# syzhang092218-source/dgppo

Hardware: AMD Instinct MI355X
Metric: env-steps/sec whole node, LidarSpread n=8 4096 envs, 1/2/4/8 GPUs (higher is better)
Workload: dtype f32

## Files before the change

### dgppo_amd/csrc/nn_dense.hip

```cpp
#include "common.h"
#include "nn_gru.h"

using f32x4 = __attribute__((ext_vector_type(4))) float;
#ifdef DGPPO_STAMPS
__device__ unsigned long long g_dstamps[32];
#define DSTAMP(i) do { if (blockIdx.x == 0 && threadIdx.x == 0) g_dstamps[i] = __builtin_amdgcn_s_memtime(); } while (0)
extern "C" int32_t dgppo_debug_stamps_dense(unsigned long long* out) {
  return (int32_t)hipMemcpyFromSymbol(out, HIP_SYMBOL(g_dstamps), sizeof(unsigned long long) * 32);
}
#else
#define DSTAMP(i)
#endif

#define DENSE_ROWS 64

struct DenseArgs {
  const float* X; int ldx;
  const float* W; int ldw;
  const float* bias;
  float* Y; int ldy;
  int M, K, N;
  int act;
  int accumulate;
  int trans_w;
// ... 201 lines not shown
    }
  } else {
    for (; tile < n_tiles; tile += gridDim.x) {
      stage_scalar(tile, 0);
      load_yold(tile);
      __syncthreads();
      compute(0);
      epilogue(tile);
      DGPPO_LDS_BARRIER();
    }
  }
#undef DGPPO_LDS_BARRIER
  DSTAMP(2);
}

template <int NTW, int RTW, int CG, int KQ, bool ACC>
static void launch_dense_acc(const DenseArgs& a, hipStream_t s) {
  constexpr int RB = 16 * RTW * (4 / CG);
  constexpr size_t smem = 2 * (size_t)RB * (KQ * 16 + 2) * sizeof(float);
  static_assert(smem <= 160 * 1024, "dense tile exceeds the 160 KB LDS of a gfx950 CU");
  static thread_local int cap = 0;
  if (cap == 0) {
    int per_cu = 0, dev = 0, cus = 256;
    if (smem > 64 * 1024)
      (void)hipFuncSetAttribute(reinterpret_cast<const void*>(&dense_fwd_kernel<NTW, RTW, CG, KQ, ACC>),
                                hipFuncAttributeMaxDynamicSharedMemorySize, (int)smem);
    if (hipOccupancyMaxActiveBlocksPerMultiprocessor(&per_cu, reinterpret_cast<const void*>(
            &dense_fwd_kernel<NTW, RTW, CG, KQ, ACC>), 256, smem) != hipSuccess || per_cu < 1) per_cu = 1;
    if (hipGetDevice(&dev) != hipSuccess ||
        hipDeviceGetAttribute(&cus, hipDeviceAttributeMultiprocessorCount, dev) != hipSuccess || cus < 1) cus = 256;
    cap = per_cu * cus;
  }
  const int n_tiles = cdiv(a.M, RB);
  const int grid = n_tiles < cap ? n_tiles : cap;
  hipLaunchKernelGGL((dense_fwd_kernel<NTW, RTW, CG, KQ, ACC>), dim3(grid), dim3(256), smem, s, a);
}

template <int NTW, int RTW, int CG, int KQ>
static void launch_dense_kq(const DenseArgs& a, hipStream_t s) {
  if (a.accumulate) launch_dense_acc<NTW, RTW, CG, KQ, true>(a, s);
  else launch_dense_acc<NTW, RTW, CG, KQ, false>(a, s);
}

template <int NTW, int RTW, int CG>
static void launch_dense(const DenseArgs& a, hipStream_t s) {
  const int kq = cdiv(a.K, 16);
  if (kq <= 1) launch_dense_kq<NTW, RTW, CG, 1>(a, s);
  else if (kq == 2) launch_dense_kq<NTW, RTW, CG, 2>(a, s);
  else if (kq == 3) launch_dense_kq<NTW, RTW, CG, 3>(a, s);
  else if (kq == 4) launch_dense_kq<NTW, RTW, CG, 4>(a, s);
  else if (kq <= 6) launch_dense_kq<NTW, RTW, CG, 6>(a, s);
  else if (kq <= 8) launch_dense_kq<NTW, RTW, CG, 8>(a, s);
  else if (kq == 9) launch_dense_kq<NTW, RTW, CG, 9>(a, s);
  else if (kq <= 12) launch_dense_kq<NTW, RTW, CG, 12>(a, s);
  else launch_dense_kq<NTW, RTW, CG, 16>(a, s);
}

#define DSK_MAXK 16
template <bool VECY>
__global__ void __launch_bounds__(256) dense_smallk_kernel(DenseArgs a) {
  __shared__ float sW[DSK_MAXK * 192 + 192];
  const int K = a.K, N = a.N, nq = (N + 3) >> 2, Nl = nq * 4;
  for (int idx = threadIdx.x; idx < K * Nl; idx += 256) {
    const int k = idx / Nl, c = idx - k * Nl;
    float w = 0.0f;
    if (c < N) w = a.trans_w ? a.W[(size_t)c * a.ldw + k] : a.W[(size_t)k * a.ldw + c];
    sW[idx] = w;
  }
  for (int c = threadIdx.x; c < Nl; c += 256) sW[K * Nl + c] = (a.bias && c < N) ? a.bias[c] : 0.0f;
  __syncthreads();
  const long items = (long)a.M * nq;
  const uint32_t rcp = (uint32_t)((0x100000000ull + nq - 1) / nq);
  for (long it = (long)blockIdx.x * 256 + threadIdx.x; it < items; it += (long)gridDim.x * 256) {
    const int row = (int)__umulhi((uint32_t)it, rcp);
    const int c0 = ((int)it - row * nq) * 4;
    const float* x = a.X + (size_t)row * a.ldx;
    float4 acc = *reinterpret_cast<const float4*>(sW + K * Nl + c0);
    for (int k = 0; k < K; ++k) {
      const float xv = x[k];
      const float4 w = *reinterpret_cast<const float4*>(sW + k * Nl + c0);
      acc.x = fmaf(xv, w.x, acc.x); acc.y = fmaf(xv, w.y, acc.y); acc.z = fmaf(xv, w.z, acc.z); acc.w = fmaf(xv, w.w, acc.w);
    }
    float* y = a.Y + (size_t)row * a.ldy + c0;
    float r[4] = {acc.x, acc.y, acc.z, acc.w};
    if (VECY) {
      if (a.accumulate) { const float4 o = *reinterpret_cast<const float4*>(y); r[0] += o.x; r[1] += o.y; r[2] += o.z; r[3] += o.w; }
      if (a.act == 1) { r[0] = relu_nan(r[0]); r[1] = relu_nan(r[1]); r[2] = relu_nan(r[2]); r[3] = relu_nan(r[3]); }
      if (a.mask) {
        const float4 mk = *reinterpret_cast<const float4*>(a.mask + (size_t)row * a.ldm + c0);
        r[0] = mk.x > 0.f ? r[0] : 0.f; r[1] = mk.y > 0.f ? r[1] : 0.f; r[2] = mk.z > 0.f ? r[2] : 0.f; r[3] = mk.w > 0.f ? r[3] : 0.f;
      }
      *reinterpret_cast<float4*>(y) = make_float4(r[0], r[1], r[2], r[3]);
    } else {
      for (int u = 0; u < 4; ++u) {
        if (c0 + u >= N) break;
        float v = r[u];
        if (a.accumulate) v += y[u];
        if (a.act == 1) v = relu_nan(v);
        if (a.mask) v = a.mask[(size_t)row * a.ldm + c0 + u] > 0.f ? v : 0.f;
        y[u] = v;
      }
    }
  }
}

static bool dense_smallk_ok(const DenseArgs& a) {
  const long nq = (a.N + 3) / 4;
  return a.K <= DSK_MAXK && a.N <= 192 && (long)a.M * nq * nq < (1l << 32);
}
static void launch_dense_smallk(const DenseArgs& a, hipStream_t s) {
  const long items = (long)a.M * ((a.N + 3) / 4);
  long blocks = (items + 256 * 4 - 1) / (256 * 4);
  blocks = blocks < 1 ? 1 : (blocks > 4096 ? 4096 : blocks);
  const bool vec = (a.N & 3) == 0 && (a.ldy & 3) == 0 && (reinterpret_cast<uintptr_t>(a.Y) & 15) == 0 &&
                   (!a.mask || ((a.ldm & 3) == 0 && (reinterpret_cast<uintptr_t>(a.mask) & 15) == 0));
  if (vec) hipLaunchKernelGGL(dense_smallk_kernel<true>, dim3((int)blocks), dim3(256), 0, s, a);
  else hipLaunchKernelGGL(dense_smallk_kernel<false>, dim3((int)blocks), dim3(256), 0, s, a);
}

int32_t dense_fwd_launch(const DenseArgs& a, hipStream_t s) {
  DGPPO_REQUIRE(a.M >= 0 && a.K >= 1 && a.N >= 1, "dense: bad shape M=%d K=%d N=%d", a.M, a.K, a.N);
  DGPPO_REQUIRE(a.N <= 192 && a.K <= 256, "dense: N <= 192 and K <= 256 supported (N=%d K=%d)", a.N, a.K);
  DGPPO_REQUIRE(a.X && a.W && a.Y, "dense: NULL operand");
  DGPPO_REQUIRE(a.ldx >= a.K && a.ldy >= a.N, "dense: leading dimensions too small");
  if (a.M == 0) return 0;
  const int nt = cdiv(a.N, 16);
  if (dense_smallk_ok(a)) launch_dense_smallk(a, s);
  else if (nt >= 9) launch_dense<3, 2, 4>(a, s);
  else if (nt >= 5) launch_dense<2, 2, 4>(a, s);
  else if (nt == 4) launch_dense<1, 2, 4>(a, s);
  else if (nt == 3) launch_dense<2, 1, 2>(a, s);
  else if (nt == 2) launch_dense<1, 1, 2>(a, s);
  else launch_dense<1, 1, 1>(a, s);
  DGPPO_LAUNCH_CHECK();
  return 0;
}

struct DenseBwdWArgs {
  const float* X; int ldx;
  const float* dY; int ldy;
  float* dW; int ldw;
  float* db;
  int M, K, N;
  int rows_per_block;
  float* part;
  int part_stride;
  size_t ws_bytes;
  const float* W; int ldwp;
  float* dX; int lddx;
  int acc_mask;
};

#define BW_ROWS 32
template <int NT, int KT, int NG, bool DX = false>
__global__ void __launch_bounds__(256 * NG) dense_bwd_w_kernel(DenseBwdWArgs a) {
  extern __shared__ float sm_wg[];
  constexpr int KTW = (KT + 3) / 4;
  constexpr int Kl = (KT & 1) ? KT * 16 : KT * 16 + 16;
  constexpr int Nl = (NT & 1) ? NT * 16 : NT * 16 + 16;
  constexpr int BUF = BW_ROWS * (Kl + Nl);
  constexpr int XQ = KT * 4, YQ = NT * 4;
  constexpr int PFX = (BW_ROWS * XQ + 255) / 256, PFY = (BW_ROWS * YQ + 255) / 256;
  const int K = a.K, N = a.N;
  const int grp = NG > 1 ? (int)(threadIdx.x >> 8) : 0;
  const int tid = threadIdx.x & 255, lane = tid & 63, wave = tid >> 6;
  const int li = lane & 15, lq = lane >> 4;
  float* sm = sm_wg + grp * 2 * BUF;
  const int wg_begin = blockIdx.x * NG * a.rows_per_block;
  const int m_begin = wg_begin + grp * a.rows_per_block;
  const int m_end = min(a.M, m_begin + a.rows_per_block);
  const int n_tiles = (min(a.M - wg_begin, a.rows_per_block) + BW_ROWS - 1) / BW_ROWS;
  const bool vec = ((K & 3) == 0) && ((a.ldx & 3) == 0) && ((reinterpret_cast<uintptr_t>(a.X) & 15) == 0) &&
                   ((N & 3) == 0) && ((a.ldy & 3) == 0) && ((reinterpret_cast<uintptr_t>(a.dY) & 15) == 0);
  const int K4 = K >> 2, N4 = N >> 2;
  f32x4 acc[KTW][NT];
#pragma unroll
  for (int i = 0; i < KTW; ++i)
#pragma unroll
    for (int t = 0; t < NT; ++t) acc[i][t] = f32x4{0.f, 0.f, 0.f, 0.f};
  float4 pfx[PFX], pfy[PFY], csum[PFY];
#pragma unroll
  for (int u = 0; u < PFY; ++u) csum[u] = make_float4(0.f, 0.f, 0.f, 0.f);
  float4 wreg[DX ? KTW : 1][DX ? NT : 1], ya[DX ? 2 : 1][DX ? NT : 1];
  if constexpr (DX) {
#pragma unroll
    for (int i = 0; i < KTW; ++i) {
      int kt = (3 - wave) + 4 * i;
      kt = kt < KT ? kt : KT - 1;
#pragma unroll
      for (int s = 0; s < NT; ++s)
        wreg[i][s] = *reinterpret_cast<const float4*>(a.W + (size_t)(kt * 16 + li) * a.ldwp + 16 * s + 4 * lq);
    }
  }
  auto fetch_a = [&](int m0) {
    if constexpr (DX) {
#pragma unroll
      for (int mt = 0; mt < 2; ++mt) {
        int row = m0 + mt * 16 + li;
        row = row < a.M ? row : a.M - 1;
#pragma unroll
        for (int s = 0; s < NT; ++s) ya[mt][s] = *reinterpret_cast<const float4*>(a.dY + (size_t)row * a.ldy + 16 * s + 4 * lq);
      }
    }
  };
  auto dx_tile = [&](int m0, int b) {
    if constexpr (DX) {
      const float* xs = sm + b * BUF;
#pragma unroll
      for (int i = 0; i < KTW; ++i) {
        const int kt = (3 - wave) + 4 * i;
        if (kt >= KT) continue;
        const int col = kt * 16 + li;
        float old[2][4];
        if (a.acc_mask) {
#pragma unroll
          for (int mt = 0; mt < 2; ++mt)
#pragma unroll
            for (int r = 0; r < 4; ++r) {
              int row = m0 + mt * 16 + lq * 4 + r;
              row = row < m_end ? row : m_end - 1;
              old[mt][r] = a.dX[(size_t)row * a.lddx + col];
            }
        }
#pragma unroll
        for (int mt = 0; mt < 2; ++mt) {
          f32x4 dx = f32x4{0.f, 0.f, 0.f, 0.f};
#pragma unroll
          for (int s = 0; s < NT; ++s) {
            dx = __builtin_amdgcn_mfma_f32_16x16x4f32(ya[mt][s].x, wreg[i][s].x, dx, 0, 0, 0);
            dx = __builtin_amdgcn_mfma_f32_16x16x4f32(ya[mt][s].y, wreg[i][s].y, dx, 0, 0, 0);
            dx = __builtin_amdgcn_mfma_f32_16x16x4f32(ya[mt][s].z, wreg[i][s].z, dx, 0, 0, 0);
            dx = __builtin_amdgcn_mfma_f32_16x16x4f32(ya[mt][s].w, wreg[i][s].w, dx, 0, 0, 0);
          }
#pragma unroll
          for (int r = 0; r < 4; ++r) {
            const int rl = mt * 16 + lq * 4 + r;
            float v = dx[r];
            if (a.acc_mask) {
              v += old[mt][r];
              v = (xs[rl * Kl + col] > 0.0f) ? v : 0.0f;
            }
            if (m0 + rl < m_end) a.dX[(size_t)(m0 + rl) * a.lddx + col] = v;
          }
        }
      }
    }
  };

  auto fetch = [&](int m0) {
#pragma unroll
    for (int u = 0; u < PFX; ++u) {
      int idx = u * 256 + tid;
      idx = idx < BW_ROWS * XQ ? idx : BW_ROWS * XQ - 1;
      const int r = idx / XQ, q = idx - r * XQ;
      int row = m0 + r;
      row = row < a.M ? row : a.M - 1;
      pfx[u] = *reinterpret_cast<const float4*>(a.X + (size_t)row * a.ldx + 4 * (q < K4 ? q : K4 - 1));
    }
#pragma unroll
    for (int u = 0; u < PFY; ++u) {
      int idx = u * 256 + tid;
      idx = idx < BW_ROWS * YQ ? idx : BW_ROWS * YQ - 1;
      const int r = idx / YQ, q = idx - r * YQ;
      int row = m0 + r;
      row = row < a.M ? row : a.M - 1;
      pfy[u] = *reinterpret_cast<const float4*>(a.dY + (size_t)row * a.ldy + 4 * (q < N4 ? q : N4 - 1));
    }
  };
  auto commit = [&](int m0, int b) {
    float* xs = sm + b * BUF;
    float* ys = xs + BW_ROWS * Kl;
#pragma unroll
    for (int u = 0; u < PFX; ++u) {
      const int idx = u * 256 + tid;
      const int r = idx / XQ, q = idx - r * XQ;
      const bool ok = (m0 + r < m_end) && (q < K4);
      const float4 v = ok ? pfx[u] : make_float4(0.f, 0.f, 0.f, 0.f);
      if (idx < BW_ROWS * XQ) *reinterpret_cast<float4*>(xs + r * Kl + 4 * q) = v;
    }
#pragma unroll
    for (int u = 0; u < PFY; ++u) {
      const int idx = u * 256 + tid;
      const int r = idx / YQ, q = idx - r * YQ;
      const bool ok = (m0 + r < m_end) && (q < N4) && (idx < BW_ROWS * YQ);
      const float4 v = ok ? pfy[u] : make_float4(0.f, 0.f, 0.f, 0.f);
      if (idx < BW_ROWS * YQ) *reinterpret_cast<float4*>(ys + r * Nl + 4 * q) = v;
      csum[u].x += v.x; csum[u].y += v.y; csum[u].z += v.z; csum[u].w += v.w;
    }
  };
  auto stage_scalar = [&](int m0) {
    float* xs = sm;
    float* ys = xs + BW_ROWS * Kl;
    for (int idx = tid; idx < BW_ROWS * KT * 16; idx += 256) {
      const int r = idx / (KT * 16), k = idx - r * (KT * 16);
      xs[r * Kl + k] = (m0 + r < m_end && k < K) ? a.X[(size_t)(m0 + r) * a.ldx + k] : 0.0f;
    }
    for (int idx = tid; idx < BW_ROWS * NT * 16; idx += 256) {
      const int r = idx / (NT * 16), c = idx - r * (NT * 16);
      ys[r * Nl + c] = (m0 + r < m_end && c < N) ? a.dY[(size_t)(m0 + r) * a.ldy + c] : 0.0f;
    }
  };
  auto compute = [&](int b) {
    const float* xs = sm + b * BUF + lq * Kl + li;
    const float* ys = sm + b * BUF + BW_ROWS * Kl + lq * Nl + li;
#pragma unroll
    for (int s4 = 0; s4 < BW_ROWS / 4; ++s4) {
      float bv[NT], av[KTW];
#pragma unroll
      for (int t = 0; t < NT; ++t) bv[t] = ys[s4 * 4 * Nl + t * 16];
#pragma unroll
      for (int i = 0; i < KTW; ++i) {
        int kt = wave + 4 * i;
        kt = kt < KT ? kt : KT - 1;
        av[i] = xs[s4 * 4 * Kl + kt * 16];
      }
#pragma unroll
      for (int i = 0; i < KTW; ++i)
#pragma unroll
        for (int t = 0; t < NT; ++t) acc[i][t] = __builtin_amdgcn_mfma_f32_16x16x4f32(av[i], bv[t], acc[i][t], 0, 0, 0);
    }
  };
#define DGPPO_LDS_BARRIER() asm volatile("s_waitcnt lgkmcnt(0)\n\ts_barrier" ::: "memory")
  float colsum = 0.0f;
  if (DX || vec) {
    fetch(m_begin);
    commit(m_begin, 0);
    __syncthreads();
    int cur = 0;
    for (int it = 0, m0 = m_begin; it < n_tiles; ++it, m0 += BW_ROWS) {
      fetch_a(m0);
      fetch(m0 + BW_ROWS);
      __builtin_amdgcn_sched_barrier(0);
      compute(cur);
      commit(m0 + BW_ROWS, cur ^ 1);
      dx_tile(m0, cur);
      DGPPO_LDS_BARRIER();
      cur ^= 1;
    }
  } else {
    for (int it = 0, m0 = m_begin; it < n_tiles; ++it, m0 += BW_ROWS) {
      stage_scalar(m0);
      __syncthreads();
      if (a.db != nullptr && tid < N) {
        const float* ys = sm + BW_ROWS * Kl;
        float cs = 0.0f;
#pragma unroll 8
        for (int r = 0; r < BW_ROWS; ++r) cs += ys[r * Nl + tid];
        colsum += cs;
      }
      compute(0);
      __syncthreads();
    }
  }
#undef DGPPO_LDS_BARRIER
  if (NG > 1) {
    constexpr int ACCF = KTW * NT * 4 * 256;
    static_assert(NG == 1 || ACCF + PFY * 4 * 256 <= 2 * BUF, "dense_bwd_w: the group exchange does not fit the tile buffers");
    __syncthreads();
    if (grp > 0) {
#pragma unroll
      for (int i = 0; i < KTW; ++i)
#pragma unroll
        for (int t = 0; t < NT; ++t)
#pragma unroll
          for (int r = 0; r < 4; ++r) sm[((i * NT + t) * 4 + r) * 256 + tid] = acc[i][t][r];
      if (!vec) csum[0].x = colsum;
#pragma unroll
      for (int u = 0; u < PFY; ++u) {
        sm[ACCF + (u * 4 + 0) * 256 + tid] = csum[u].x; sm[ACCF + (u * 4 + 1) * 256 + tid] = csum[u].y;
        sm[ACCF + (u * 4 + 2) * 256 + tid] = csum[u].z; sm[ACCF + (u * 4 + 3) * 256 + tid] = csum[u].w;
      }
    }
    __syncthreads();
    if (grp == 0) {
      for (int g = 1; g < NG; ++g) {
        const float* o = sm_wg + g * 2 * BUF;
#pragma unroll
        for (int i = 0; i < KTW; ++i)
#pragma unroll
          for (int t = 0; t < NT; ++t)
#pragma unroll
            for (int r = 0; r < 4; ++r) acc[i][t][r] += o[((i * NT + t) * 4 + r) * 256 + tid];
        if (!vec) colsum += o[ACCF + tid];
        else {
#pragma unroll
          for (int u = 0; u < PFY; ++u) {
            csum[u].x += o[ACCF + (u * 4 + 0) * 256 + tid]; csum[u].y += o[ACCF + (u * 4 + 1) * 256 + tid];
            csum[u].z += o[ACCF + (u * 4 + 2) * 256 + tid]; csum[u].w += o[ACCF + (u * 4 + 3) * 256 + tid];
          }
        }
      }
    }
  }
  float* slab = a.part ? a.part + (size_t)blockIdx.x * a.part_stride : nullptr;
#pragma unroll
  for (int i = 0; i < KTW; ++i) {
    const int kt = wave + 4 * i;
    if (kt >= KT || grp != 0) continue;
#pragma unroll
    for (int t = 0; t < NT; ++t) {
      const int col = t * 16 + li;
      if (col >= N) continue;
#pragma unroll
      for (int r = 0; r < 4; ++r) {
        const int krow = kt * 16 + lq * 4 + r;
        if (krow >= K) continue;
        if (slab) slab[krow * N + col] = acc[i][t][r];
        else atomicAdd(a.dW + (size_t)krow * a.ldw + col, acc[i][t][r]);
      }
    }
  }
  if (a.db != nullptr) {
    float cs = colsum;
    if (vec) {
      __syncthreads();
      float* red = sm;
#pragma unroll
      for (int u = 0; u < PFY; ++u) {
        const int idx = u * 256 + tid;
        const int r = idx / YQ, q = idx - r * YQ;
        if (idx < BW_ROWS * YQ) *reinterpret_cast<float4*>(red + r * (YQ * 4) + 4 * q) = csum[u];
      }
      __syncthreads();
      cs = 0.0f;
      if (tid < N) {
#pragma unroll 8
        for (int r = 0; r < BW_ROWS; ++r) cs += red[r * (YQ * 4) + tid];
      }
    }
    if (tid < N && grp == 0) {
      if (slab) slab[K * N + tid] = cs;
      else atomicAdd(a.db + tid, cs);
    }
  }
}

#define REDUCE_SLABS_PER_SPLIT 16

__global__ void __launch_bounds__(256) dense_bwd_w_reduce_kernel(const float* __restrict__ part, int part_stride, int G,
                                                                 float* __restrict__ dW, int ldw, float* __restrict__ db,
                                                                 int K, int N) {
  const int e = blockIdx.x * 256 + threadIdx.x;
  const int E = K * N + (db ? N : 0);
  if (e >= E) return;
  const int per = (G + gridDim.y - 1) / gridDim.y;
  const int g0 = blockIdx.y * per, g1 = min(G, g0 + per);
  float s0 = 0.f, s1 = 0.f, s2 = 0.f, s3 = 0.f;
  int g = g0;
  for (; g + 3 < g1; g += 4) {
    s0 += part[(size_t)g * part_stride + e];
    s1 += part[(size_t)(g + 1) * part_stride + e];
    s2 += part[(size_t)(g + 2) * part_stride + e];
    s3 += part[(size_t)(g + 3) * part_stride + e];
  }
  for (; g < g1; ++g) s0 += part[(size_t)g * part_stride + e];
  const float sum = (s0 + s1) + (s2 + s3);
  if (g0 >= g1) return;
  if (e < K * N) {
    const int k = e / N, n = e - k * N;
    atomicAdd(dW + (size_t)k * ldw + n, sum);
  } else {
    atomicAdd(db + (e - K * N), sum);
  }
}

static thread_local dgppo_reduce_desc* g_defer = nullptr;

struct ReduceBatch {
  int n;
  dgppo_reduce_desc d[DGPPO_REDUCE_BATCH];
};

__global__ void __launch_bounds__(256) dense_bwd_w_reduce_batch_kernel(ReduceBatch b) {
  const dgppo_reduce_desc& d = b.d[blockIdx.z];
  const int K = d.K, N = d.N, G = d.slabs;
  const int e = blockIdx.x * 256 + threadIdx.x;
  const int E = K * N + (d.db ? N : 0);
  if (e >= E) return;
  const int splits = min((int)gridDim.y, max(1, (G + REDUCE_SLABS_PER_SPLIT - 1) / REDUCE_SLABS_PER_SPLIT));
  if ((int)blockIdx.y >= splits) return;
  const int per = (G + splits - 1) / splits;
  const int g0 = blockIdx.y * per, g1 = min(G, g0 + per);
  if (g0 >= g1) return;
  const float* part = d.part;
  const size_t st = (size_t)d.part_stride;
  float s0 = 0.f, s1 = 0.f, s2 = 0.f, s3 = 0.f;
  int g = g0;
  for (; g + 3 < g1; g += 4) {
    s0 += part[(size_t)g * st + e]; s1 += part[(size_t)(g + 1) * st + e];
    s2 += part[(size_t)(g + 2) * st + e]; s3 += part[(size_t)(g + 3) * st + e];
  }
  for (; g < g1; ++g) s0 += part[(size_t)g * st + e];
  const float sum = (s0 + s1) + (s2 + s3);
  if (e < K * N) {
    const int k = e / N, n = e - k * N;
    atomicAdd(d.dW + (size_t)k * d.ldw + n, sum);
  } else {
    atomicAdd(d.db + (e - K * N), sum);
  }
}

static void reduce_or_defer(hipStream_t s, const float* part, int stride, int grid, float* dW, int ldw, float* db, int K, int N) {
  if (g_defer != nullptr) {
    dgppo_reduce_desc& d = *g_defer;
    d.part = part; d.part_stride = stride; d.slabs = grid; d.dW = dW; d.ldw = ldw; d.db = db; d.K = K; d.N = N; d.pending = 1;
    return;
  }
  const int E = K * N + (db ? N : 0);
  int splits = cdiv(grid, REDUCE_SLABS_PER_SPLIT);
  splits = splits < 1 ? 1 : (splits > 64 ? 64 : splits);
  hipLaunchKernelGGL(dense_bwd_w_reduce_kernel, dim3(cdiv(E, 256), splits), dim3(256), 0, s, part, stride, grid, dW, ldw, db, K, N);
}

static int device_cus() {
  static thread_local int cus = 0;
  if (cus == 0) {
    int dev = 0;
    if (hipGetDevice(&dev) != hipSuccess ||
        hipDeviceGetAttribute(&cus, hipDeviceAttributeMultiprocessorCount, dev) != hipSuccess || cus < 1) cus = 256;
  }
  return cus;
}

template <int NT, int KT>
constexpr int bwd_w_groups() {
  constexpr int KTW = (KT + 3) / 4;
  constexpr int Kl = (KT & 1) ? KT * 16 : KT * 16 + 16;
  constexpr int Nl = (NT & 1) ? NT * 16 : NT * 16 + 16;
  constexpr int BUF2 = 2 * BW_ROWS * (Kl + Nl);
  constexpr int PFY = (BW_ROWS * NT * 4 + 255) / 256;
  constexpr int fit = (160 * 1024) / (BUF2 * 4);
  constexpr bool xch = KTW * NT * 4 * 256 + PFY * 4 * 256 <= BUF2;
  return (!xch || fit < 2) ? 1 : (fit > 4 ? 4 : fit);
}

template <int NT, int KT, bool DX = false, int NGX = 0>
static void launch_bwd_w_kt(DenseBwdWArgs a, hipStream_t s) {
  constexpr int Kl = (KT & 1) ? KT * 16 : KT * 16 + 16;
  constexpr int Nl = (NT & 1) ? NT * 16 : NT * 16 + 16;
  constexpr size_t smem = 2 * sizeof(float) * BW_ROWS * (Kl + Nl);
  constexpr int NG = NGX > 0 ? NGX : bwd_w_groups<NT, KT>();
  static_assert(NG <= bwd_w_groups<NT, KT>(), "dense_bwd_w: more groups than the tile buffers and their exchange allow");
  static_assert(smem * NG <= 160 * 1024, "dense_bwd_w tiles exceed the 160 KB LDS of a gfx950 CU");
  static thread_local bool opted = false;
  if (!opted) {
    if (smem > 64 * 1024)
      (void)hipFuncSetAttribute(reinterpret_cast<const void*>(&dense_bwd_w_kernel<NT, KT, 1, DX>),
                                hipFuncAttributeMaxDynamicSharedMemorySize, (int)smem);
    if (NG > 1 && smem * NG > 64 * 1024)
      (void)hipFuncSetAttribute(reinterpret_cast<const void*>(&dense_bwd_w_kernel<NT, KT, NG, DX>),
                                hipFuncAttributeMaxDynamicSharedMemorySize, (int)(smem * NG));
    opted = true;
  }
  const int cus = device_cus();
  int rpb = cdiv(a.M, NG * cus);
  rpb = ((rpb + BW_ROWS - 1) / BW_ROWS) * BW_ROWS;
  if (rpb < 2 * BW_ROWS) rpb = 2 * BW_ROWS;
  const int ng = cdiv(a.M, rpb) > cus ? NG : 1;
  const int stride = ((a.K * a.N + a.N + 63) / 64) * 64;
  const size_t ws_bytes = a.ws_bytes;
  float* ws = cdiv(a.M, rpb) > 4 ? a.part : nullptr;
  if (ws) {
    const long max_slabs = (long)(ws_bytes / (sizeof(float) * stride));
    if (max_slabs < 8) ws = nullptr;
    else if (cdiv(a.M, rpb * ng) > max_slabs) rpb = ((cdiv(a.M, (int)max_slabs * ng) + BW_ROWS - 1) / BW_ROWS) * BW_ROWS;
  }
  a.rows_per_block = rpb;
  a.part = ws;
  a.part_stride = stride;
  const int grid = cdiv(a.M, rpb * ng);
  if (NG > 1 && ng > 1) hipLaunchKernelGGL((dense_bwd_w_kernel<NT, KT, NG, DX>), dim3(grid), dim3(256 * NG), smem * NG, s, a);
  else hipLaunchKernelGGL((dense_bwd_w_kernel<NT, KT, 1, DX>), dim3(grid), dim3(256), smem, s, a);
  if (ws) reduce_or_defer(s, ws, stride, grid, a.dW, a.ldw, a.db, a.K, a.N);
}

template <int NT>
static void launch_bwd_w(const DenseBwdWArgs& a, hipStream_t s) {
  const int kt = cdiv(a.K, 16);
  if (kt <= 1) launch_bwd_w_kt<NT, 1>(a, s);
  else if (kt == 2) launch_bwd_w_kt<NT, 2>(a, s);
  else if (kt == 3) launch_bwd_w_kt<NT, 3>(a, s);
  else if (kt == 4) launch_bwd_w_kt<NT, 4>(a, s);
  else if (kt <= 6) launch_bwd_w_kt<NT, 6>(a, s);
  else if (kt <= 8) launch_bwd_w_kt<NT, 8>(a, s);
  else if (kt == 9) launch_bwd_w_kt<NT, 9>(a, s);
  else if (kt <= 12) launch_bwd_w_kt<NT, 12>(a, s);
  else launch_bwd_w_kt<NT, 16>(a, s);
}

template <int KMAX, bool VECX>
__global__ void __launch_bounds__(256) dense_bwd_w_smallk_kernel(DenseBwdWArgs a) {
  extern __shared__ float sP[];
  const int K = a.K, N = a.N, nq = N >> 2;
  const int per = K * 4 + 4, Pl = per + 1;
  const int lanes = 256 / nq;
  const int rl = threadIdx.x / nq, cq = threadIdx.x - rl * nq;
  float4 acc[KMAX];
#pragma unroll
  for (int k = 0; k < KMAX; ++k) acc[k] = make_float4(0.f, 0.f, 0.f, 0.f);
  float4 accb = make_float4(0.f, 0.f, 0.f, 0.f);
  if (rl < lanes) {
    const int r0 = blockIdx.x * a.rows_per_block;
    const int r1 = min(a.M, r0 + a.rows_per_block);
    constexpr int UR = 4;
    for (int rb = r0 + rl; rb < r1; rb += lanes * UR) {
      float4 d[UR];
      float xv[UR][KMAX];
#pragma unroll
      for (int u = 0; u < UR; ++u) {
        const int r = rb + u * lanes;
        const bool in = r < r1;
        const int rr = in ? r : r0;
        d[u] = *reinterpret_cast<const float4*>(a.dY + (size_t)rr * a.ldy + cq * 4);
        if (!in) d[u] = make_float4(0.f, 0.f, 0.f, 0.f);
        const float* x = a.X + (size_t)rr * a.ldx;
        if (VECX) {
#pragma unroll
          for (int k4 = 0; k4 < KMAX / 4; ++k4) {
            if (k4 * 4 < K) {
              const float4 t = *reinterpret_cast<const float4*>(x + k4 * 4);
              xv[u][k4 * 4] = t.x; xv[u][k4 * 4 + 1] = t.y; xv[u][k4 * 4 + 2] = t.z; xv[u][k4 * 4 + 3] = t.w;
            }
          }
        } else {
#pragma unroll
          for (int k = 0; k < KMAX; ++k) if (k < K) xv[u][k] = x[k];
        }
      }
#pragma unroll
      for (int u = 0; u < UR; ++u) {
        accb.x += d[u].x; accb.y += d[u].y; accb.z += d[u].z; accb.w += d[u].w;
#pragma unroll
        for (int k = 0; k < KMAX; ++k) {
          if (k < K) {
            acc[k].x = fmaf(xv[u][k], d[u].x, acc[k].x); acc[k].y = fmaf(xv[u][k], d[u].y, acc[k].y);
            acc[k].z = fmaf(xv[u][k], d[u].z, acc[k].z); acc[k].w = fmaf(xv[u][k], d[u].w, acc[k].w);
          }
        }
      }
    }
  }
  float* mine = sP + threadIdx.x * Pl;
#pragma unroll
  for (int k = 0; k < KMAX; ++k) {
    if (k < K) { mine[k * 4] = acc[k].x; mine[k * 4 + 1] = acc[k].y; mine[k * 4 + 2] = acc[k].z; mine[k * 4 + 3] = acc[k].w; }
  }
  mine[K * 4] = accb.x; mine[K * 4 + 1] = accb.y; mine[K * 4 + 2] = accb.z; mine[K * 4 + 3] = accb.w;
  __syncthreads();
  float* out = a.part + (size_t)blockIdx.x * a.part_stride;
  const int E = K * N + N;
  for (int e = threadIdx.x; e < E; e += 256) {
    const int k = e / N, c = e - k * N;
    const float* src = sP + (c >> 2) * Pl + k * 4 + (c & 3);
    float s0 = 0.f, s1 = 0.f;
    int l = 0;
    for (; l + 1 < lanes; l += 2) { s0 += src[(size_t)l * nq * Pl]; s1 += src[(size_t)(l + 1) * nq * Pl]; }
    if (l < lanes) s0 += src[(size_t)l * nq * Pl];
    out[e] = s0 + s1;
  }
}

static bool launch_bwd_w_smallk(DenseBwdWArgs a, hipStream_t s) {
  if (a.K > 16 || a.N > 64 || (a.N & 3) || (a.ldy & 3) || (reinterpret_cast<uintptr_t>(a.dY) & 15) || a.M < 4096)
    return false;
  const int stride = ((a.K * a.N + a.N + 63) / 64) * 64;
  const long max_slabs = a.part ? (long)(a.ws_bytes / (sizeof(float) * stride)) : 0;
  if (max_slabs < 8) return false;
  int grid = a.M >= (1 << 19) ? 1024 : 512;
  if (grid > max_slabs) grid = (int)max_slabs;
  int rpb = cdiv(a.M, grid);
  grid = cdiv(a.M, rpb);
  a.rows_per_block = rpb;
  a.part_stride = stride;
  const size_t smem = sizeof(float) * 256 * (a.K * 4 + 5);
  const bool vx = (a.K & 3) == 0 && (a.ldx & 3) == 0 && (reinterpret_cast<uintptr_t>(a.X) & 15) == 0;
  if (a.K <= 8) {
    if (vx) hipLaunchKernelGGL((dense_bwd_w_smallk_kernel<8, true>), dim3(grid), dim3(256), smem, s, a);
    else hipLaunchKernelGGL((dense_bwd_w_smallk_kernel<8, false>), dim3(grid), dim3(256), smem, s, a);
  } else {
    static thread_local bool opted = false;
    if (!opted) {
      (void)hipFuncSetAttribute(reinterpret_cast<const void*>(&dense_bwd_w_smallk_kernel<16, true>),
                                hipFuncAttributeMaxDynamicSharedMemorySize, 256 * 69 * 4);
      (void)hipFuncSetAttribute(reinterpret_cast<const void*>(&dense_bwd_w_smallk_kernel<16, false>),
                                hipFuncAttributeMaxDynamicSharedMemorySize, 256 * 69 * 4);
      opted = true;
    }
    if (vx) hipLaunchKernelGGL((dense_bwd_w_smallk_kernel<16, true>), dim3(grid), dim3(256), smem, s, a);
    else hipLaunchKernelGGL((dense_bwd_w_smallk_kernel<16, false>), dim3(grid), dim3(256), smem, s, a);
  }
  reduce_or_defer(s, a.part, stride, grid, a.dW, a.ldw, a.db, a.K, a.N);
  return true;
}

int32_t dense_bwd_w_launch(DenseBwdWArgs a, hipStream_t s) {
  DGPPO_REQUIRE(a.M >= 0 && a.K >= 1 && a.N >= 1, "dense_bwd_w: bad shape");
  DGPPO_REQUIRE(a.N <= 192 && a.K <= 256, "dense_bwd_w: N <= 192 and K <= 256 supported (N=%d K=%d)", a.N, a.K);
  DGPPO_REQUIRE(a.X && a.dY && a.dW, "dense_bwd_w: NULL operand");
  DGPPO_REQUIRE(a.ldx >= a.K && a.ldy >= a.N && a.ldw >= a.N, "dense_bwd_w: leading dimensions too small");
  if (a.M == 0) return 0;
  const int nt = cdiv(a.N, 16);
  if (launch_bwd_w_smallk(a, s)) {}
  else if (nt <= 1) launch_bwd_w<1>(a, s);
  else if (nt <= 2) launch_bwd_w<2>(a, s);
  else if (nt <= 4) launch_bwd_w<4>(a, s);
  else if (nt <= 6) launch_bwd_w<6>(a, s);
  else launch_bwd_w<12>(a, s);
  DGPPO_LAUNCH_CHECK();
  return 0;
}

struct XwSite { int K, N, NT, KT, NG; };
constexpr XwSite kXwSites[] = {{144, 64, 4, 9, 2}, {48, 32, 2, 3, 4}, {48, 64, 4, 3, 2}};
constexpr int kXwSiteCount = sizeof(kXwSites) / sizeof(kXwSites[0]);

static bool bwd_w_vec(const DenseBwdWArgs& a) {
  return (a.K & 3) == 0 && (a.ldx & 3) == 0 && (reinterpret_cast<uintptr_t>(a.X) & 15) == 0 && (a.N & 3) == 0 && (a.ldy & 3) == 0 &&
         (reinterpret_cast<uintptr_t>(a.dY) & 15) == 0;
}

static bool bwd_xw_fused(const DenseBwdWArgs& a) {
  bool site = false;
  for (int i = 0; i < kXwSiteCount; ++i) site = site || (a.K == kXwSites[i].K && a.N == kXwSites[i].N);
  const uintptr_t p = reinterpret_cast<uintptr_t>(a.W) | reinterpret_cast<uintptr_t>(a.dX);
  return site && a.N <= 192 && bwd_w_vec(a) && ((a.ldwp | a.lddx) & 3) == 0 && (p & 15) == 0;
}

template <int I>
static void launch_xw_site(const DenseBwdWArgs& a, hipStream_t s) {
  if constexpr (I < kXwSiteCount) {
    constexpr XwSite S = kXwSites[I];
    static_assert(S.K == S.KT * 16 && S.N == S.NT * 16, "dense_bwd_xw: a site is whole 16-wide tiles (W^T and dY fragments are unguarded)");
    if (a.K == S.K && a.N == S.N) launch_bwd_w_kt<S.NT, S.KT, true, S.NG>(a, s);
    else launch_xw_site<I + 1>(a, s);
  }
}

static int32_t dense_bwd_xw_launch(DenseBwdWArgs a, hipStream_t s) {
  DGPPO_REQUIRE(a.M >= 0 && a.K >= 1 && a.N >= 1, "dense_bwd_xw: bad shape");
  DGPPO_REQUIRE(a.X && a.dY && a.dW && a.W && a.dX, "dense_bwd_xw: NULL operand");
  DGPPO_REQUIRE(a.ldx >= a.K && a.ldy >= a.N && a.ldw >= a.N && a.ldwp >= a.N && a.lddx >= a.K,
                "dense_bwd_xw: leading dimensions too small");
  if (a.M == 0) return 0;
  if (!bwd_xw_fused(a)) {
    const int32_t rc = dense_bwd_w_launch(a, s);
    if (rc) return rc;
    DenseArgs f{a.dY, a.ldy, a.W, a.ldwp, nullptr, a.dX, a.lddx, a.M, a.N, a.K, 0, a.acc_mask, 1, a.acc_mask ? a.X : nullptr, a.ldx};
    return dense_fwd_launch(f, s);
  }
  launch_xw_site<0>(a, s);
  DGPPO_LAUNCH_CHECK();
  return 0;
}

#define GW_AL 144
#define GW_YL 272
#define GW_BUF (BW_ROWS * (GW_AL + GW_YL))
#define GW_SLAB_WI 0
#define GW_SLAB_BI (64 * 192)
#define GW_SLAB_WH (64 * 192 + 192)
#define GW_SLAB_BHN (2 * 64 * 192 + 192)
#define GW_SLAB (2 * 64 * 192 + 192 + 64)
struct GruBwdWArgs {
  const float* x; int ldx;
  const float* hprev; int ldh;
  const float* dgi;
  const float* dhn;
  float* dWi; int ldwi;
  float* dbi;
  float* dWh; int ldwh;
  float* dbhn;
  int M, rows_per_block;
  float* part;
  const float* dhs;
  const float* gates;
  float* dgi_out;
};

template <bool T1>
__global__ void __launch_bounds__(512) gru_bwd_w_kernel(GruBwdWArgs a) {
  extern __shared__ float sm[];
  const int tid = threadIdx.x, lane = tid & 63, wave = (tid >> 6) & 3, half = tid >> 8;
  const int li = lane & 15, lq = lane >> 4;
  const int m_begin = blockIdx.x * a.rows_per_block;
  const int m_end = min(a.M, m_begin + a.rows_per_block);
  f32x4 acc[12];
#pragma unroll
  for (int t = 0; t < 12; ++t) acc[t] = f32x4{0.f, 0.f, 0.f, 0.f};
  float4 pfa[2], pfy[T1 ? 6 : 4];
  float4 csum[T1 ? 4 : 1];
#pragma unroll
  for (int u = 0; u < (T1 ? 4 : 1); ++u) csum[u] = make_float4(0.f, 0.f, 0.f, 0.f);
  const int qa = tid & 31, ra = tid >> 5, qy = tid & 63, ry = tid >> 6;
  const int q1 = tid & 15, r1 = tid >> 4;
  auto fetch = [&](int m0) {
#pragma unroll
    for (int u = 0; u < 2; ++u) {
      int row = m0 + u * 16 + ra;
      row = row < a.M ? row : a.M - 1;
      const float* src = qa < 16 ? a.x + (size_t)row * a.ldx + 4 * qa : a.hprev + (size_t)row * a.ldh + 4 * (qa - 16);
      pfa[u] = *reinterpret_cast<const float4*>(src);
    }
    if constexpr (T1) {
      int row = m0 + r1;
      row = row < a.M ? row : a.M - 1;
      pfy[0] = *reinterpret_cast<const float4*>(a.dhs + (size_t)row * 64 + 4 * q1);
      pfy[1] = *reinterpret_cast<const float4*>(a.hprev + (size_t)row * a.ldh + 4 * q1);
      const float* gs = a.gates + (size_t)row * 256 + 4 * q1;
#pragma unroll
      for (int g = 0; g < 4; ++g) pfy[2 + g] = *reinterpret_cast<const float4*>(gs + 64 * g);
    } else {
#pragma unroll
      for (int u = 0; u < 4; ++u) {
        int row = m0 + u * 8 + ry;
        row = row < a.M ? row : a.M - 1;
        const float* src = qy < 48 ? a.dgi + (size_t)row * 192 + 4 * qy : a.dhn + (size_t)row * 64 + 4 * (qy - 48);
        pfy[u] = *reinterpret_cast<const float4*>(src);
      }
    }
  };
  auto commit = [&](int m0, int b) {
    float* as = sm + b * GW_BUF;
    float* ys = as + BW_ROWS * GW_AL;
#pragma unroll
    for (int u = 0; u < 2; ++u) {
      const int r = u * 16 + ra;
      const float4 v = (m0 + r < m_end) ? pfa[u] : make_float4(0.f, 0.f, 0.f, 0.f);
      *reinterpret_cast<float4*>(as + r * GW_AL + 4 * qa) = v;
    }
    if constexpr (T1) {
      const bool in = m0 + r1 < m_end;
      const GruGateGrad g0 = gru_gate_grad(gru_zero_carry(pfy[0].x), pfy[1].x, pfy[2].x, pfy[3].x, pfy[4].x, pfy[5].x);
      const GruGateGrad g1 = gru_gate_grad(gru_zero_carry(pfy[0].y), pfy[1].y, pfy[2].y, pfy[3].y, pfy[4].y, pfy[5].y);
      const GruGateGrad g2 = gru_gate_grad(gru_zero_carry(pfy[0].z), pfy[1].z, pfy[2].z, pfy[3].z, pfy[4].z, pfy[5].z);
      const GruGateGrad g3 = gru_gate_grad(gru_zero_carry(pfy[0].w), pfy[1].w, pfy[2].w, pfy[3].w, pfy[4].w, pfy[5].w);
      float4 v[4] = {make_float4(g0.dar, g1.dar, g2.dar, g3.dar), make_float4(g0.daz, g1.daz, g2.daz, g3.daz),
                     make_float4(g0.dan, g1.dan, g2.dan, g3.dan), make_float4(g0.dhn, g1.dhn, g2.dhn, g3.dhn)};
      if (in) {
        float* o = a.dgi_out + (size_t)(m0 + r1) * 192 + 4 * q1;
#pragma unroll
        for (int g = 0; g < 3; ++g) *reinterpret_cast<float4*>(o + 64 * g) = v[g];
      }
#pragma unroll
      for (int g = 0; g < 4; ++g) {
        if (!in) v[g] = make_float4(0.f, 0.f, 0.f, 0.f);
        *reinterpret_cast<float4*>(ys + r1 * GW_YL + 64 * g + 4 * q1) = v[g];
        csum[g].x += v[g].x; csum[g].y += v[g].y; csum[g].z += v[g].z; csum[g].w += v[g].w;
      }
    } else {
#pragma unroll
      for (int u = 0; u < 4; ++u) {
        const int r = u * 8 + ry;
        const float4 v = (m0 + r < m_end) ? pfy[u] : make_float4(0.f, 0.f, 0.f, 0.f);
        *reinterpret_cast<float4*>(ys + r * GW_YL + 4 * qy) = v;
        csum[0].x += v.x; csum[0].y += v.y; csum[0].z += v.z; csum[0].w += v.w;
      }
    }
  };
  auto compute = [&](int b) {
    const float* as = sm + b * GW_BUF + lq * GW_AL + half * 64 + wave * 16 + li;
    const float* ys = sm + b * GW_BUF + BW_ROWS * GW_AL + lq * GW_YL + li;
    const float* yh = ys + (half ? 64 : 0);
#pragma unroll
    for (int s4 = 0; s4 < BW_ROWS / 4; ++s4) {
      float bv[12];
#pragma unroll
      for (int t = 0; t < 8; ++t) bv[t] = ys[s4 * 4 * GW_YL + t * 16];
#pragma unroll
      for (int t = 8; t < 12; ++t) bv[t] = yh[s4 * 4 * GW_YL + t * 16];
      const float av = as[s4 * 4 * GW_AL];
#pragma unroll
      for (int t = 0; t < 12; ++t) acc[t] = __builtin_amdgcn_mfma_f32_16x16x4f32(av, bv[t], acc[t], 0, 0, 0);
    }
  };
  fetch(m_begin);
  commit(m_begin, 0);
  __syncthreads();
  int cur = 0;
  for (int m0 = m_begin; m0 < m_end; m0 += BW_ROWS) {
    fetch(m0 + BW_ROWS);
    __builtin_amdgcn_sched_barrier(0);
    compute(cur);
    commit(m0 + BW_ROWS, cur ^ 1);
    asm volatile("s_waitcnt lgkmcnt(0)\n\ts_barrier" ::: "memory");
    cur ^= 1;
  }
  float* slab = a.part ? a.part + (size_t)blockIdx.x * GW_SLAB : nullptr;
// ... 186 lines not shown
```

Measured before the change: 4.661 million.

## Restructure fused dense backward dX: wave work dealing, LDS-staged coalesced stores, new site

Reworks the fused weight-grad plus input-grad backward kernel. dX tiles are now split evenly across waves in 16x16 units, using dY fragments read from the already-staged LDS buffer instead of separate global loads. Results are staged in an extra LDS buffer and written out as coalesced float4 rows one iteration later, overlapping with the next tile. The accumulate/mask path becomes a compile-time template with vector loads of the old dX values, waves that own surplus dX work skip one weight-grad k-tile, and a new fused site (K=32, N=96) is added. This costs extra LDS per group and more template instances, and adds complexity around the deferred-store edge handling.

```diff
diff --git a/dgppo_amd/csrc/nn_dense.hip b/dgppo_amd/csrc/nn_dense.hip
--- a/dgppo_amd/csrc/nn_dense.hip
+++ b/dgppo_amd/csrc/nn_dense.hip
@@ -377,7 +377,23 @@
 };
 
 #define BW_ROWS 32
-template <int NT, int KT, int NG, bool DX = false>
+template <int KT>
+struct XwDeal {
+  static constexpr int nkt(int w) { return w < KT ? (KT - w + 3) / 4 : 0; }
+  static constexpr int units(int w) { return KT - 2 * nkt(w); }
+  static constexpr int start(int w) { int s = 0; for (int v = 0; v < w; ++v) s += units(v); return s; }
+  static constexpr int kw() {
+    int m = 1;
+    for (int w = 0; w < 4; ++w) {
+      const int k = units(w) > 0 ? ((start(w) + units(w) - 1) >> 1) - (start(w) >> 1) + 1 : 0;
+      m = k > m ? k : m;
+    }
+    return m;
+  }
+};
+#define XW_DL(KT) ((KT) * 16 + 4)
+
+template <int NT, int KT, int NG, bool DX = false, bool ACCM = false>
 __global__ void __launch_bounds__(256 * NG) dense_bwd_w_kernel(DenseBwdWArgs a) {
   extern __shared__ float sm_wg[];
   constexpr int KTW = (KT + 3) / 4;
@@ -406,76 +422,103 @@
   float4 pfx[PFX], pfy[PFY], csum[PFY];
 #pragma unroll
   for (int u = 0; u < PFY; ++u) csum[u] = make_float4(0.f, 0.f, 0.f, 0.f);
-  float4 wreg[DX ? KTW : 1][DX ? NT : 1], ya[DX ? 2 : 1][DX ? NT : 1];
+  using D = XwDeal<KT>;
+  constexpr int KW = DX ? D::kw() : 1;
+  constexpr int Dl = XW_DL(KT);
+  const int wv = __builtin_amdgcn_readfirstlane(wave);
+  const int u0 = wv == 0 ? D::start(0) : wv == 1 ? D::start(1) : wv == 2 ? D::start(2) : D::start(3);
+  const int u1 = u0 + (wv == 0 ? D::units(0) : wv == 1 ? D::units(1) : wv == 2 ? D::units(2) : D::units(3));
+  const int kb = u0 >> 1;
+  float* dxs = sm_wg + NG * 2 * BUF + grp * BW_ROWS * Dl;
+  float4 wreg[KW][DX ? NT : 1], old[ACCM ? KW : 1][ACCM ? 2 : 1];
   if constexpr (DX) {
-#pragma unroll
-    for (int i = 0; i < KTW; ++i) {
-      int kt = (3 - wave) + 4 * i;
-      kt = kt < KT ? kt : KT - 1;
+    static_assert(KT >= 2 && D::start(3) + D::units(3) == 2 * KT, "dense_bwd_xw: the waves' units cover the dX tile");
+#pragma unroll
+    for (int c = 0; c < KW; ++c) {
+      const int kt = kb + c < KT ? kb + c : KT - 1;
 #pragma unroll
       for (int s = 0; s < NT; ++s)
-        wreg[i][s] = *reinterpret_cast<const float4*>(a.W + (size_t)(kt * 16 + li) * a.ldwp + 16 * s + 4 * lq);
-    }
-  }
-  auto fetch_a = [&](int m0) {
-    if constexpr (DX) {
+        wreg[c][s] = *reinterpret_cast<const float4*>(a.W + (size_t)(kt * 16 + li) * a.ldwp + 16 * s + 4 * lq);
+    }
+  }
+  auto fetch_old = [&](int m0) {
+    if constexpr (ACCM) {
 #pragma unroll
       for (int mt = 0; mt < 2; ++mt) {
         int row = m0 + mt * 16 + li;
         row = row < a.M ? row : a.M - 1;
 #pragma unroll
-        for (int s = 0; s < NT; ++s) ya[mt][s] = *reinterpret_cast<const float4*>(a.dY + (size_t)row * a.ldy + 16 * s + 4 * lq);
-      }
-    }
-  };
-  auto dx_tile = [&](int m0, int b) {
+        for (int c = 0; c < KW; ++c) {
+          const int u = 2 * (kb + c) + mt;
+          if (u >= u0 && u < u1) old[c][mt] = *reinterpret_cast<const float4*>(a.dX + (size_t)row * a.lddx + (kb + c) * 16 + 4 * lq);
+        }
+      }
+    }
+  };
+  auto dx_tile = [&](int b) {
     if constexpr (DX) {
-      const float* xs = sm + b * BUF;
-#pragma unroll
-      for (int i = 0; i < KTW; ++i) {
-        const int kt = (3 - wave) + 4 * i;
-        if (kt >= KT) continue;
-        const int col = kt * 16 + li;
-        float old[2][4];
-        if (a.acc_mask) {
-#pragma unroll
-          for (int mt = 0; mt < 2; ++mt)
-#pragma unroll
-            for (int r = 0; r < 4; ++r) {
-              int row = m0 + mt * 16 + lq * 4 + r;
-              row = row < m_end ? row : m_end - 1;
-              old[mt][r] = a.dX[(size_t)row * a.lddx + col];
-            }
+      [[maybe_unused]] const float* xs = sm + b * BUF;
+      if (u1 == u0) return;
+      const float* ys = sm + b * BUF + BW_ROWS * Kl + li * Nl + 4 * lq;
+      f32x4 ya[2][NT];
+#pragma unroll
+      for (int mt = 0; mt < 2; ++mt)
+#pragma unroll
+        for (int s = 0; s < NT; ++s) ya[mt][s] = *reinterpret_cast<const f32x4*>(ys + mt * 16 * Nl + 16 * s);
+#pragma unroll
+      for (int c = 0; c < KW; ++c)
+#pragma unroll
+        for (int mt = 0; mt < 2; ++mt) {
+          const int u = 2 * (kb + c) + mt;
+          if (u < u0 || u >= u1) continue;
+          f32x4 dx = f32x4{0.f, 0.f, 0.f, 0.f};
+#pragma unroll
+          for (int s = 0; s < NT; ++s) {
+            dx = __builtin_amdgcn_mfma_f32_16x16x4f32(wreg[c][s].x, ya[mt][s][0], dx, 0, 0, 0);
+            dx = __builtin_amdgcn_mfma_f32_16x16x4f32(wreg[c][s].y, ya[mt][s][1], dx, 0, 0, 0);
+            dx = __builtin_amdgcn_mfma_f32_16x16x4f32(wreg[c][s].z, ya[mt][s][2], dx, 0, 0, 0);
+            dx = __builtin_amdgcn_mfma_f32_16x16x4f32(wreg[c][s].w, ya[mt][s][3], dx, 0, 0, 0);
+          }
+          const int rl = mt * 16 + li, col = (kb + c) * 16 + 4 * lq;
+          if constexpr (ACCM) {
+            const float4 x = *reinterpret_cast<const float4*>(xs + rl * Kl + col);
+            const float4 o = old[c][mt];
+            dx[0] = (x.x > 0.0f) ? o.x + dx[0] : 0.0f; dx[1] = (x.y > 0.0f) ? o.y + dx[1] : 0.0f;
+            dx[2] = (x.z > 0.0f) ? o.z + dx[2] : 0.0f; dx[3] = (x.w > 0.0f) ? o.w + dx[3] : 0.0f;
+          }
+          *reinterpret_cast<f32x4*>(dxs + rl * Dl + col) = dx;
         }
-#pragma unroll
-        for (int mt = 0; mt < 2; ++mt) {
-          f32x4 dx = f32x4{0.f, 0.f, 0.f, 0.f};
-#pragma unroll
-          for (int s = 0; s < NT; ++s) {
-            dx = __builtin_amdgcn_mfma_f32_16x16x4f32(ya[mt][s].x, wreg[i][s].x, dx, 0, 0, 0);
-            dx = __builtin_amdgcn_mfma_f32_16x16x4f32(ya[mt][s].y, wreg[i][s].y, dx, 0, 0, 0);
-            dx = __builtin_amdgcn_mfma_f32_16x16x4f32(ya[mt][s].z, wreg[i][s].z, dx, 0, 0, 0);
-            dx = __builtin_amdgcn_mfma_f32_16x16x4f32(ya[mt][s].w, wreg[i][s].w, dx, 0, 0, 0);
-          }
-#pragma unroll
-          for (int r = 0; r < 4; ++r) {
-            const int rl = mt * 16 + lq * 4 + r;
-            float v = dx[r];
-            if (a.acc_mask) {
-              v += old[mt][r];
-              v = (xs[rl * Kl + col] > 0.0f) ? v : 0.0f;
-            }
-            if (m0 + rl < m_end) a.dX[(size_t)(m0 + rl) * a.lddx + col] = v;
-          }
-        }
-      }
-    }
-  };
-
+    }
+  };
+#define DGPPO_LDS_BARRIER() asm volatile("s_waitcnt lgkmcnt(0)\n\ts_barrier" ::: "memory")
+  auto rows_out = [&](int m0, bool in_loop) {
+    if constexpr (DX) {
+      constexpr int RPP = 256 / XQ, NP = (BW_ROWS + RPP - 1) / RPP;
+      const int r0 = tid / XQ, q = tid - r0 * XQ;
+      const bool lane_ok = r0 < RPP;
+      const float* src = dxs + (lane_ok ? r0 : 0) * Dl + 4 * q;
+      f32x4 q4[NP];
+#pragma unroll
+      for (int u = 0; u < NP; ++u)
+        q4[u] = *reinterpret_cast<const f32x4*>(src + (u * RPP + RPP <= BW_ROWS ? u * RPP : BW_ROWS - RPP) * Dl);
+      if (in_loop) DGPPO_LDS_BARRIER();
+      float* dst = a.dX + (size_t)(m0 + r0) * a.lddx + 4 * q;
+#pragma unroll
+      for (int u = 0; u < NP; ++u) {
+        constexpr int kShift = NP * RPP - BW_ROWS;
+        const int r = (u == NP - 1 ? u * RPP - kShift : u * RPP) + r0;
+        const bool fresh = u < NP - 1 || r0 >= kShift;
+        if (lane_ok && fresh && m0 + r >= m_begin && m0 + r < m_end)
+          *reinterpret_cast<f32x4*>(dst + (ptrdiff_t)(u == NP - 1 ? u * RPP - kShift : u * RPP) * a.lddx) = q4[u];
+      }
+    }
+  };
+
+  int tl = tid;
   auto fetch = [&](int m0) {
 #pragma unroll
     for (int u = 0; u < PFX; ++u) {
-      int idx = u * 256 + tid;
+      int idx = u * 256 + tl;
       idx = idx < BW_ROWS * XQ ? idx : BW_ROWS * XQ - 1;
       const int r = idx / XQ, q = idx - r * XQ;
       int row = m0 + r;
@@ -484,7 +527,7 @@
     }
 #pragma unroll
     for (int u = 0; u < PFY; ++u) {
-      int idx = u * 256 + tid;
+      int idx = u * 256 + tl;
       idx = idx < BW_ROWS * YQ ? idx : BW_ROWS * YQ - 1;
       const int r = idx / YQ, q = idx - r * YQ;
       int row = m0 + r;
@@ -497,7 +540,7 @@
     float* ys = xs + BW_ROWS * Kl;
 #pragma unroll
     for (int u = 0; u < PFX; ++u) {
-      const int idx = u * 256 + tid;
+      const int idx = u * 256 + tl;
       const int r = idx / XQ, q = idx - r * XQ;
       const bool ok = (m0 + r < m_end) && (q < K4);
       const float4 v = ok ? pfx[u] : make_float4(0.f, 0.f, 0.f, 0.f);
@@ -505,7 +548,7 @@
     }
 #pragma unroll
     for (int u = 0; u < PFY; ++u) {
-      const int idx = u * 256 + tid;
+      const int idx = u * 256 + tl;
       const int r = idx / YQ, q = idx - r * YQ;
       const bool ok = (m0 + r < m_end) && (q < N4) && (idx < BW_ROWS * YQ);
       const float4 v = ok ? pfy[u] : make_float4(0.f, 0.f, 0.f, 0.f);
@@ -525,27 +568,27 @@
       ys[r * Nl + c] = (m0 + r < m_end && c < N) ? a.dY[(size_t)(m0 + r) * a.ldy + c] : 0.0f;
     }
   };
+#define DGPPO_BW_COMPUTE(NA)                                                                                                  \
+  _Pragma("unroll") for (int s4 = 0; s4 < BW_ROWS / 4; ++s4) {                                                                \
+    float bv[NT], av[(NA) > 0 ? (NA) : 1];                                                                                    \
+    _Pragma("unroll") for (int t = 0; t < NT; ++t) bv[t] = ys[s4 * 4 * Nl + t * 16];                                         \
+    _Pragma("unroll") for (int i = 0; i < (NA); ++i) {                                                                        \
+      int kt = wave + 4 * i;                                                                                                  \
+      kt = kt < KT ? kt : KT - 1;                                  \
+      av[i] = xs[s4 * 4 * Kl + kt * 16];                                                                                      \
+    }                                                                                                                         \
+    _Pragma("unroll") for (int i = 0; i < (NA); ++i)                                                                          \
+      _Pragma("unroll") for (int t = 0; t < NT; ++t)                                                                          \
+        acc[i][t] = __builtin_amdgcn_mfma_f32_16x16x4f32(av[i], bv[t], acc[i][t], 0, 0, 0);                                   \
+  }
+  const bool surplus = DX && wv + 4 * (KTW - 1) >= KT;
   auto compute = [&](int b) {
     const float* xs = sm + b * BUF + lq * Kl + li;
     const float* ys = sm + b * BUF + BW_ROWS * Kl + lq * Nl + li;
-#pragma unroll
-    for (int s4 = 0; s4 < BW_ROWS / 4; ++s4) {
-      float bv[NT], av[KTW];
-#pragma unroll
-      for (int t = 0; t < NT; ++t) bv[t] = ys[s4 * 4 * Nl + t * 16];
-#pragma unroll
-      for (int i = 0; i < KTW; ++i) {
-        int kt = wave + 4 * i;
-        kt = kt < KT ? kt : KT - 1;
-        av[i] = xs[s4 * 4 * Kl + kt * 16];
-      }
-#pragma unroll
-      for (int i = 0; i < KTW; ++i)
-#pragma unroll
-        for (int t = 0; t < NT; ++t) acc[i][t] = __builtin_amdgcn_mfma_f32_16x16x4f32(av[i], bv[t], acc[i][t], 0, 0, 0);
-    }
-  };
-#define DGPPO_LDS_BARRIER() asm volatile("s_waitcnt lgkmcnt(0)\n\ts_barrier" ::: "memory")
+    if (DX && surplus) { DGPPO_BW_COMPUTE(KTW - 1) }
+    else { DGPPO_BW_COMPUTE(KTW) }
+  };
+#undef DGPPO_BW_COMPUTE
   float colsum = 0.0f;
   if (DX || vec) {
     fetch(m_begin);
@@ -553,15 +596,19 @@
     __syncthreads();
     int cur = 0;
     for (int it = 0, m0 = m_begin; it < n_tiles; ++it, m0 += BW_ROWS) {
-      fetch_a(m0);
+      if constexpr (DX) asm volatile("" : "+v"(tl));
+      rows_out(m0 - BW_ROWS, true);
+      if constexpr (DX) __builtin_amdgcn_sched_barrier(0);
+      fetch_old(m0);
       fetch(m0 + BW_ROWS);
       __builtin_amdgcn_sched_barrier(0);
       compute(cur);
       commit(m0 + BW_ROWS, cur ^ 1);
-      dx_tile(m0, cur);
+      dx_tile(cur);
       DGPPO_LDS_BARRIER();
       cur ^= 1;
     }
+    rows_out(m_begin + (n_tiles - 1) * BW_ROWS, false);
   } else {
     for (int it = 0, m0 = m_begin; it < n_tiles; ++it, m0 += BW_ROWS) {
       stage_scalar(m0);
@@ -759,21 +806,21 @@
   return (!xch || fit < 2) ? 1 : (fit > 4 ? 4 : fit);
 }
 
-template <int NT, int KT, bool DX = false, int NGX = 0>
+template <int NT, int KT, bool DX = false, int NGX = 0, bool ACCM = false>
 static void launch_bwd_w_kt(DenseBwdWArgs a, hipStream_t s) {
   constexpr int Kl = (KT & 1) ? KT * 16 : KT * 16 + 16;
   constexpr int Nl = (NT & 1) ? NT * 16 : NT * 16 + 16;
-  constexpr size_t smem = 2 * sizeof(float) * BW_ROWS * (Kl + Nl);
+  constexpr size_t smem = sizeof(float) * BW_ROWS * (2 * (Kl + Nl) + (DX ? XW_DL(KT) : 0));
   constexpr int NG = NGX > 0 ? NGX : bwd_w_groups<NT, KT>();
   static_assert(NG <= bwd_w_groups<NT, KT>(), "dense_bwd_w: more groups than the tile buffers and their exchange allow");
   static_assert(smem * NG <= 160 * 1024, "dense_bwd_w tiles exceed the 160 KB LDS of a gfx950 CU");
   static thread_local bool opted = false;
   if (!opted) {
     if (smem > 64 * 1024)
-      (void)hipFuncSetAttribute(reinterpret_cast<const void*>(&dense_bwd_w_kernel<NT, KT, 1, DX>),
+      (void)hipFuncSetAttribute(reinterpret_cast<const void*>(&dense_bwd_w_kernel<NT, KT, 1, DX, ACCM>),
                                 hipFuncAttributeMaxDynamicSharedMemorySize, (int)smem);
     if (NG > 1 && smem * NG > 64 * 1024)
-      (void)hipFuncSetAttribute(reinterpret_cast<const void*>(&dense_bwd_w_kernel<NT, KT, NG, DX>),
+      (void)hipFuncSetAttribute(reinterpret_cast<const void*>(&dense_bwd_w_kernel<NT, KT, NG, DX, ACCM>),
                                 hipFuncAttributeMaxDynamicSharedMemorySize, (int)(smem * NG));
     opted = true;
   }
@@ -794,8 +841,8 @@
   a.part = ws;
   a.part_stride = stride;
   const int grid = cdiv(a.M, rpb * ng);
-  if (NG > 1 && ng > 1) hipLaunchKernelGGL((dense_bwd_w_kernel<NT, KT, NG, DX>), dim3(grid), dim3(256 * NG), smem * NG, s, a);
-  else hipLaunchKernelGGL((dense_bwd_w_kernel<NT, KT, 1, DX>), dim3(grid), dim3(256), smem, s, a);
+  if (NG > 1 && ng > 1) hipLaunchKernelGGL((dense_bwd_w_kernel<NT, KT, NG, DX, ACCM>), dim3(grid), dim3(256 * NG), smem * NG, s, a);
+  else hipLaunchKernelGGL((dense_bwd_w_kernel<NT, KT, 1, DX, ACCM>), dim3(grid), dim3(256), smem, s, a);
   if (ws) reduce_or_defer(s, ws, stride, grid, a.dW, a.ldw, a.db, a.K, a.N);
 }
 
@@ -935,8 +982,8 @@
   return 0;
 }
 
-struct XwSite { int K, N, NT, KT, NG; };
-constexpr XwSite kXwSites[] = {{144, 64, 4, 9, 2}, {48, 32, 2, 3, 4}, {48, 64, 4, 3, 2}};
+struct XwSite { int K, N, NT, KT, NG; bool ACC; };
+constexpr XwSite kXwSites[] = {{144, 64, 4, 9, 2, false}, {48, 32, 2, 3, 4, true}, {48, 64, 4, 3, 2, true}, {32, 96, 6, 2, 2, true}};
 constexpr int kXwSiteCount = sizeof(kXwSites) / sizeof(kXwSites[0]);
 
 static bool bwd_w_vec(const DenseBwdWArgs& a) {
@@ -946,7 +993,7 @@
 
 static bool bwd_xw_fused(const DenseBwdWArgs& a) {
   bool site = false;
-  for (int i = 0; i < kXwSiteCount; ++i) site = site || (a.K == kXwSites[i].K && a.N == kXwSites[i].N);
+  for (int i = 0; i < kXwSiteCount; ++i) site = site || (a.K == kXwSites[i].K && a.N == kXwSites[i].N && (kXwSites[i].ACC || !a.acc_mask));
   const uintptr_t p = reinterpret_cast<uintptr_t>(a.W) | reinterpret_cast<uintptr_t>(a.dX);
   return site && a.N <= 192 && bwd_w_vec(a) && ((a.ldwp | a.lddx) & 3) == 0 && (p & 15) == 0;
 }
@@ -956,8 +1003,9 @@
   if constexpr (I < kXwSiteCount) {
     constexpr XwSite S = kXwSites[I];
     static_assert(S.K == S.KT * 16 && S.N == S.NT * 16, "dense_bwd_xw: a site is whole 16-wide tiles (W^T and dY fragments are unguarded)");
-    if (a.K == S.K && a.N == S.N) launch_bwd_w_kt<S.NT, S.KT, true, S.NG>(a, s);
-    else launch_xw_site<I + 1>(a, s);
+    if (a.K != S.K || a.N != S.N) launch_xw_site<I + 1>(a, s);
+    else if (!a.acc_mask) launch_bwd_w_kt<S.NT, S.KT, true, S.NG, false>(a, s);
+    else if constexpr (S.ACC) launch_bwd_w_kt<S.NT, S.KT, true, S.NG, true>(a, s);
   }
 }
 
```

Measured after the change: 4.798 million (median of 6 runs). 2.9% higher.
